# Aceinna/gnss-ins-sim

Measured on NVIDIA H100. Metric: MC-runs x timesteps/sec free_integration @100Hz, higher is better.
Workload: dtype f64

## Files before the change

### gnss_ins_sim_b200/csrc/b2ins_api.cu

```cuda
#include <cmath>
#include <cstdarg>
#include <cstdio>
#include <cstdlib>
#include <cstring>
#include <limits>
#include <vector>

#include "../../include/b2ins.h"
#include "allan_kernel.cuh"
#include "internal.h"
#include "noise_kernel.cuh"
#include "pathgen_host.h"
#include "psd_kernel.cuh"
#include "gps_kernel.cuh"
#include "ekf_kernel.cuh"
#include "stats_kernel.cuh"

#ifdef B2INS_SINGLE_TU
#define B2_RF 0
#define B2_PLAIN_NAME launch_mc_plain_rf0
#define B2_SPEC_NAME launch_mc_spec_rf0
#include "mc_plain_launch.cuh"
#include "mc_spec_launch.cuh"
#undef B2_RF
// ... 933 lines not shown
  if (rc != B2INS_OK) return rc;
  CU_CHECK(cudaMemcpyAsync(avar, dav.p, static_cast<size_t>(nseries) * ntau * sizeof(double),
                           cudaMemcpyDeviceToHost, st.s));
  CU_CHECK(cudaMemcpyAsync(tau, dtau.p, static_cast<size_t>(ntau) * sizeof(double),
                           cudaMemcpyDeviceToHost, st.s));
  CU_CHECK(cudaStreamSynchronize(st.s));
  return B2INS_OK;
}

int b2ins_psd_series_len(int64_t n) { return n > 0 ? psd_series_len(n) : 0; }

int64_t b2ins_psd_workspace_bytes(int64_t n, int64_t runs) {
  if (n <= 0 || runs <= 0) return 16;
  const int64_t L = psd_series_len(n) / 2 + 1;
  return runs * 3 * L * 2 * static_cast<int64_t>(sizeof(double)) + 8192 * 16 + 64;
}

int b2ins_psd_series_f64(double fs, int64_t n, int64_t runs, int sensor, int table_len,
                         const double* freq, const double* sxx3, uint64_t seed,
                         int64_t run_offset, double* series, void* workspace, void* stream) {
  ARG_CHECK(fs > 0.0 && n > 0 && runs >= 0, "bad fs/n/runs");
  ARG_CHECK(sensor == 0 || sensor == 1, "sensor must be 0 (accel) or 1 (gyro)");
  ARG_CHECK(table_len >= 2, "the PSD table needs at least two rows");
  if (runs == 0) return B2INS_OK;
  ARG_CHECK(freq && sxx3 && series && workspace, "null buffer");
  ARG_CHECK(runs * 3 <= 65535, "at most 21845 runs per call (grid.y)");
  PsdParams p;
  p.fs = fs;
  p.runs = runs;
  p.run_offset = run_offset;
  p.N = psd_series_len(n);
  p.L = p.N / 2 + 1;
  p.L0 = table_len;
  p.sensor = sensor;
  p.interp = (table_len != p.L) ? 1 : 0;
  p.k0 = static_cast<uint32_t>(seed);
  p.k1 = static_cast<uint32_t>(seed >> 32);
  p.freq = freq;
  p.sxx = sxx3;
  p.ab = static_cast<double*>(workspace);
  p.series = series;
  cudaStream_t s = static_cast<cudaStream_t>(stream);
  dim3 g1((p.L + kPsdThreads - 1) / kPsdThreads, static_cast<unsigned>(runs * 3));
  psd_phase_kernel<<<g1, kPsdThreads, 0, s>>>(p);
  int bluestein = 0;
  static const bool no_fft = std::getenv("B2INS_PSD_DIRECT") != nullptr;
  const int P = no_fft ? 0 : psd_fft_plan(p.N, &bluestein);
  if (P == 0) {
    dim3 g2((p.N + kPsdThreads - 1) / kPsdThreads, static_cast<unsigned>(runs * 3));
    psd_synth_kernel<<<g2, kPsdThreads, 0, s>>>(p);
    CU_CHECK(cudaGetLastError());
    return B2INS_OK;
  }
  PsdFftParams f;
  f.nseries = runs * 3;
  f.N = p.N;
  f.L = p.L;
  f.M = p.N / 2;
  f.P = P;
  f.logP = 0;
  while ((1 << f.logP) < P) ++f.logP;
  f.bluestein = bluestein;
  f.ab = p.ab;
  uintptr_t tail = reinterpret_cast<uintptr_t>(p.ab + runs * 3 * static_cast<int64_t>(p.L) * 2);
  tail = (tail + 15) & ~static_cast<uintptr_t>(15);
  f.bhat = reinterpret_cast<double2*>(tail);
  f.series = series;
  const size_t smem = static_cast<size_t>(P) * 16 + static_cast<size_t>(P / 2) * 16;
  static int attr_dev = -1;
  int dev = 0;
  CU_CHECK(cudaGetDevice(&dev));
  if (attr_dev != dev) {
    CU_CHECK(cudaFuncSetAttribute(psd_fft_kernel, cudaFuncAttributeMaxDynamicSharedMemorySize, 8192 * 24));
    CU_CHECK(cudaFuncSetAttribute(psd_chirp_kernel, cudaFuncAttributeMaxDynamicSharedMemorySize, 8192 * 24));
    attr_dev = dev;
  }
  if (bluestein) psd_chirp_kernel<<<1, kFftThreads, smem, s>>>(f);
  const int64_t grid = f.nseries < 2 * sm_count() ? f.nseries : 2 * sm_count();
  psd_fft_kernel<<<static_cast<unsigned>(grid), kFftThreads, smem, s>>>(f);
  CU_CHECK(cudaGetLastError());
  return B2INS_OK;
}

int64_t b2ins_path_rows(const double* motion_def, int64_t segs, double fs) {
  if (!motion_def || segs <= 0 || !(fs > 0.0)) return -1;
  return b2ins_host::path_rows(motion_def, segs, fs);
}

int64_t b2ins_path_gen_host(const double* ini, const double* motion_def, int64_t segs, double fs,
                            double osr, double fs_gps, double fs_odo, const double* mobility,
                            int ref_frame, int64_t cap, double* imu, double* nav, double* gps,
                            int64_t* gps_rows, double* odo) {
  if (!ini || !motion_def || !mobility || !imu || !nav || segs <= 0 || !(fs > 0.0) || !(osr >= 1.0) ||
      (ref_frame != 0 && ref_frame != 1) || (gps && !(fs_gps > 0.0))) {
    fail(B2INS_ERR_ARG, "bad argument to b2ins_path_gen_host");
    return -1;
  }
  return b2ins_host::path_gen(ini, motion_def, segs, fs, osr, fs_gps, fs_odo, mobility, ref_frame,
                              cap, imu, nav, gps, gps_rows, odo);
}

__global__ void dfma_rate_kernel(double* out, int iters) {
  double a0 = threadIdx.x * 1e-9, a1 = a0 + 1, a2 = a0 + 2, a3 = a0 + 3, a4 = a0 + 4,
         a5 = a0 + 5, a6 = a0 + 6, a7 = a0 + 7;
  const double m = 1.0000001, c = 1e-9;
  for (int i = 0; i < iters; ++i) {
    a0 = fma(a0, m, c); a1 = fma(a1, m, c); a2 = fma(a2, m, c); a3 = fma(a3, m, c);
    a4 = fma(a4, m, c); a5 = fma(a5, m, c); a6 = fma(a6, m, c); a7 = fma(a7, m, c);
  }
  out[static_cast<size_t>(blockIdx.x) * blockDim.x + threadIdx.x] = a0 + a1 + a2 + a3 + a4 + a5 + a6 + a7;
}

int b2ins_diag_auto_lanes(int64_t runs, int fused, int sm_count_arg) {
  return auto_lanes(runs < 1 ? 1 : runs, fused != 0, sm_count_arg);
}

int b2ins_diag_mc_shape(int lanes_per_run, int ref_frame, int* shape3) {
  ARG_CHECK(shape3, "null output");
  ARG_CHECK(lanes_per_run == 1 || lanes_per_run == 2 || lanes_per_run == 4 || lanes_per_run == 8 ||
                lanes_per_run == 16 || lanes_per_run == 32, "lanes_per_run must be 1,2,4,8,16 or 32");
  McShape sh = default_shape(lanes_per_run, ref_frame);
  shape_override(&sh);
  shape3[0] = sh.spec ? sh.P : 0;
  shape3[1] = sh.spec ? sh.WI : 0;
  shape3[2] = (sh.spec && sh.split) ? 1 : 0;
  return B2INS_OK;
}

int b2ins_diag_dfma_rate(double* dfma_per_s) {
  ARG_CHECK(dfma_per_s, "null output");
  const int blocks = sm_count() * 8, threads = 256, iters = 8000;
  DevBuf out;
  CU_CHECK(out.alloc(sizeof(double) * blocks * threads));
  cudaEvent_t e0, e1;
  CU_CHECK(cudaEventCreate(&e0));
  CU_CHECK(cudaEventCreate(&e1));
  float best = 1e30f;
  for (int rep = 0; rep < 4; ++rep) {
    CU_CHECK(cudaEventRecord(e0, nullptr));
    dfma_rate_kernel<<<blocks, threads>>>(out.d(), iters);
    CU_CHECK(cudaEventRecord(e1, nullptr));
    CU_CHECK(cudaEventSynchronize(e1));
    float ms = 0.f;
    CU_CHECK(cudaEventElapsedTime(&ms, e0, e1));
    if (rep > 0 && ms < best) best = ms;
  }
  cudaEventDestroy(e0);
  cudaEventDestroy(e1);
  *dfma_per_s = static_cast<double>(blocks) * threads * iters * 8.0 / (best * 1e-3);
  return B2INS_OK;
}

#ifdef B2INS_PHASE_CLOCKS
int b2ins_diag_phase_clocks(unsigned long long* out8, int reset) {
  if (out8) cudaMemcpyFromSymbol(out8, g_phase_clocks, sizeof(unsigned long long) * 8);
  if (reset) {
    unsigned long long z[8] = {0, 0, 0, 0, 0, 0, 0, 0};
    cudaMemcpyToSymbol(g_phase_clocks, z, sizeof(z));
  }
  return B2INS_OK;
}
#endif

}
```

### gnss_ins_sim_b200/csrc/mc_av_kernel.cuh

```cuda
#pragma once
#include "mc_spec_kernel.cuh"

namespace b2ins {

constexpr int kAvRound = 8;
template <int G>
struct AvShape {
  static constexpr int kHalves = (32 / G) / 4;
  static constexpr int kProd = 6 * kHalves;
  static constexpr int kWarps = (G == 4) ? 16 : 12;
  static constexpr int kSync = 32 * (2 + kProd);
};
__device__ constexpr int kAvRole8[12] = {-1, -2, 0, 1, -3, 2, 3, 4, -3, 5, -3, -3};
__device__ constexpr int kAvRole4[16] = {-1, -2, 0, 1, 2, 3, 4, 5, -3, 6, 7, 8, -3, 9, 10, 11};

template <int G>
struct AvSmem {
  alignas(128) double gyro[kStagesFast][kTile * 3];
  alignas(128) double accel[kStagesFast][kTile * 3];
  alignas(16) SampleSlot slot[3][kAvRound / G][32];
  alignas(16) double ring[2][kAvRound][32 / G][6];
  alignas(8) uint64_t full[kStagesFast];
  alignas(8) uint64_t empty[kStagesFast];
};

template <int G>
__global__ void __launch_bounds__(AvShape<G>::kWarps * 32, 1) mc_av_kernel(const __grid_constant__ McParams p) {
  static_assert(G == 4 || G == 8, "groups of 4 or 8 lanes");
  constexpr int kRunsPerCta = 32 / G;
  constexpr int kProd = AvShape<G>::kProd;
  constexpr int kAvSync = AvShape<G>::kSync;
  __shared__ AvSmem<G> sm;
  const int lane = threadIdx.x & 31;
  const int pwarp = threadIdx.x >> 5;
  const int role_w = (G == 4) ? kAvRole4[pwarp] : kAvRole8[pwarp];
  const bool is_a = role_w == -1, is_v = role_w == -2, is_p = role_w >= 0;
  const int pp = is_p ? role_w : 0;
  const int j = is_p ? (lane & 7) : lane % G;
  const int grp = is_p ? (pp / 6) * 4 + (lane >> 3) : lane / G;
  const int64_t run_raw = static_cast<int64_t>(blockIdx.x) * kRunsPerCta + grp;
  const bool active = run_raw < p.runs;
  const int64_t run = active ? run_raw : p.runs - 1;
  const int64_t grun = p.run_offset + run;
  const uint32_t run_lo = static_cast<uint32_t>(grun), run_hi = static_cast<uint32_t>(grun >> 32);
  const bool dump = active && run < p.dump_runs;
  const bool warp_dumps = __any_sync(0xffffffffu, dump);
  const int64_t num_tiles = (p.n + kTile - 1) / kTile;
  const int issuer = 2 * 32;
  auto stage_sync = [&]() { asm volatile("bar.sync 1, %0;" ::"n"(kAvSync) : "memory"); };

  if (threadIdx.x == 0) {
    for (int s = 0; s < kStagesFast; ++s) {
      mbar_init(&sm.full[s], 1);
      mbar_init(&sm.empty[s], kProd);
    }
    mbar_fence_init();
  }
  __syncthreads();
  if (!is_a && !is_v && !is_p) return;
  const int64_t rounds = (p.n + kAvRound - 1) / kAvRound;

  if (is_p) {
    if (threadIdx.x == issuer)
      for (int s = 0; s < kStagesFast && s < num_tiles; ++s) spec_issue_tile(sm, p, s, s);
    const int c = pp % 6, ax = c % 3;
    const bool is_acc = c < 3;
    const TriadNoise& e = is_acc ? p.accel : p.gyro;
    double carry = 0.0;
    const double apj = ipow(e.gm_a[ax], j), aG = ipow(e.gm_a[ax], kAvRound);
    double phase[3] = {0.0, 0.0, 0.0};
    if (p.gyro.vib_type == 2) {
#pragma unroll
      for (int k = 0; k < 3; ++k)
        phase[k] = (uniform01(0xFFFFFFFFu, kDrawPhase + k, run_lo, run_hi, p.k0, p.k1) * 2.0) * kPi;
    }
    const bool any_vib = (p.accel.vib_type | p.gyro.vib_type) != 0;
    for (int64_t i = 0; i < rounds + 2; ++i) {
      if (i < rounds) {
        const int64_t r0 = i * kAvRound;
        const int64_t tile = r0 / kTile;
        const int s = static_cast<int>(tile % kStagesFast);
        const int base = static_cast<int>(r0 - tile * kTile);
        const int cnt = static_cast<int>(min64(kTile, p.n - tile * kTile));
        if (base == 0) {
          if (threadIdx.x == issuer && tile >= 1 && tile - 1 + kStagesFast < num_tiles) {
            const int sp = static_cast<int>((tile - 1) % kStagesFast);
            mbar_wait(&sm.empty[sp], static_cast<uint32_t>(((tile - 1) / kStagesFast) & 1));
            spec_issue_tile(sm, p, tile - 1 + kStagesFast, sp);
          }
          mbar_wait(&sm.full[s], static_cast<uint32_t>((tile / kStagesFast) & 1));
        }
        const int buf = static_cast<int>(i % 3);
        {
          const int tj = base + j;
          const int64_t t = tile * kTile + tj;
          const bool live = tj < cnt;
          Normal2 z{0.0, 0.0};
          double m = 0.0;
          if (live) {
            z = normal_pair(static_cast<uint32_t>(t), c, run_lo, run_hi, p.k0, p.k1);
            const double ref = is_acc ? sm.accel[s][tj * 3 + ax] : sm.gyro[s][tj * 3 + ax];
            m = (ref + e.b[ax]) + e.w[ax] * z.z1;
            if (any_vib)
              m += vib_term(e, ax, is_acc ? 0 : 1, static_cast<uint32_t>(t), run_lo, run_hi, p.k0, p.k1, run, phase);
          }
          const double d = gm_block<kAvRound>(e.gm_b[ax] * z.z0, e.gm_a[ax], apj, aG, j, carry);
          m += d + e.wd[ax] * z.z0;
          int64_t row;
          if (warp_dumps && dump && live && p.out_gyro && dump_row(p, t, &row))
            (is_acc ? p.out_accel : p.out_gyro)[run * p.osr + row * p.ost + ax * p.osc] = m;
          SampleSlot& mine = sm.slot[buf][j / G][grp * G + (j % G)];
          if (is_acc) mine.a[ax] = m; else mine.g[ax] = m;
        }
        if (base + kAvRound >= cnt) {
          __syncwarp();
          if (lane == 0) mbar_arrive(&sm.empty[s]);
        }
      }
      if (i <= rounds) stage_sync();
    }
    return;
  }

  NavState st0;
  {
    const int64_t irun = p.ini_offset + run;
    const int64_t set = (irun < p.ini_sets) ? irun : 0;
    nav_init<1>(st0, p.ini + set * p.ini_rows, p.ini_rows, p.dt);
  }

  if (is_a) {
    AttState a;
    a.yaw = st0.yaw; a.pitch = st0.pitch; a.roll = st0.roll;
    a.sc = st0.sc;
    a.icp = st0.icp;
    if (dump && j == 0 && p.out_att) {
      const int64_t o = run * p.osr;
      p.out_att[o] = a.yaw;
      p.out_att[o + p.osc] = a.pitch;
      p.out_att[o + 2 * p.osc] = a.roll;
      if (p.out_quat) write_quat(p.out_quat + run * p.dump_rows * 4, a.yaw, a.pitch, a.roll);
    }
    for (int64_t i = 0; i < rounds + 2; ++i) {
      if (i >= 1 && i <= rounds) {
        const int64_t r0 = (i - 1) * kAvRound;
        const int sbuf = static_cast<int>((i - 1) % 3), rbuf = static_cast<int>((i - 1) & 1);
        const int kmax = static_cast<int>(min64(kAvRound, p.n - 1 - r0));
        auto a_step = [&](int k) {
          const SampleSlot& sl = sm.slot[sbuf][k / G][lane - j + (k % G)];
          const Vec3 w{sl.g[0], sl.g[1], sl.g[2]};
          att_step(a, w, p.dt, ((r0 + k + 1) & (kResync - 1)) == 0);
          if (j == 0) {
            double* o = sm.ring[rbuf][k][grp];
            reinterpret_cast<double2*>(o)[0] = make_double2(a.sc.sy, a.sc.cy);
            reinterpret_cast<double2*>(o)[1] = make_double2(a.sc.sp, a.sc.cp);
            reinterpret_cast<double2*>(o)[2] = make_double2(a.sc.sr, a.sc.cr);
          }
          int64_t row;
          if (warp_dumps && dump && j == 0 && p.out_att && dump_row(p, r0 + k + 1, &row)) {
            const int64_t o = run * p.osr + row * p.ost;
            const double y = wrap_once(a.yaw), r = wrap_once(a.roll);
            p.out_att[o] = y;
            p.out_att[o + p.osc] = a.pitch;
            p.out_att[o + 2 * p.osc] = r;
            if (p.out_quat) write_quat(p.out_quat + (run * p.dump_rows + row) * 4, y, a.pitch, r);
          }
        };
        if (warp_dumps || kmax < kAvRound) {
#pragma unroll 1
          for (int k = 0; k < kmax; ++k) a_step(k);
        } else {
#pragma unroll 1
          for (int kb = 0; kb < kAvRound; kb += 4) {
            bool redo = ((r0 + kb) & (kResync - 1)) + 4 >= kResync;
            if (!redo) {
              const AttState saved = a;
              bool cold = false;
#pragma unroll
              for (int k = 0; k < 4; ++k) {
                const SampleSlot& sl = sm.slot[sbuf][(kb + k) / G][lane - j + ((kb + k) % G)];
                const Vec3 w{sl.g[0], sl.g[1], sl.g[2]};
                cold |= att_step<true>(a, w, p.dt, false);
                if (j == 0) {
                  double* o = sm.ring[rbuf][kb + k][grp];
                  reinterpret_cast<double2*>(o)[0] = make_double2(a.sc.sy, a.sc.cy);
                  reinterpret_cast<double2*>(o)[1] = make_double2(a.sc.sp, a.sc.cp);
                  reinterpret_cast<double2*>(o)[2] = make_double2(a.sc.sr, a.sc.cr);
                }
              }
              redo = __any_sync(0xffffffffu, cold);
              if (__builtin_expect(redo, 0)) a = saved;
            }
            if (redo) {
#pragma unroll 1
              for (int k = 0; k < 4; ++k) a_step(kb + k);
            }
          }
        }
      }
      if (i <= rounds) stage_sync();
    }
    if (active && j == 0) {
      const double* r = p.ref_nav + (p.n - 1) * 9;
      if (p.end_err) {
        double* e = p.end_err + run * 9;
        e[0] = angle_range_pi(a.yaw - r[0]);
        e[1] = angle_range_pi(a.pitch - r[1]);
        e[2] = angle_range_pi(a.roll - r[2]);
      }
      if (p.end_state) {
        double* e = p.end_state + run * 9;
        e[0] = wrap_once(a.yaw); e[1] = a.pitch; e[2] = wrap_once(a.roll);
      }
    }
    return;
  }

  VelState v;
  v.vel_b = st0.vel_b;
  v.vel = st0.vel;
  v.pos = st0.pos;
  v.gdt = st0.g * p.dt;
  SinCos3 old = st0.sc;
  if (dump && j == 0 && p.out_att) {
    const int64_t o = run * p.osr;
    p.out_pos[o] = v.pos.x;
    p.out_pos[o + p.osc] = v.pos.y;
    p.out_pos[o + 2 * p.osc] = v.pos.z;
    p.out_vel[o] = v.vel.x;
    p.out_vel[o + p.osc] = v.vel.y;
    p.out_vel[o + 2 * p.osc] = v.vel.z;
  }
  for (int64_t i = 0; i < rounds + 2; ++i) {
    if (i >= 2) {
      const int64_t r0 = (i - 2) * kAvRound;
      const int sbuf = static_cast<int>((i - 2) % 3), rbuf = static_cast<int>((i - 2) & 1);
      const int kmax = static_cast<int>(min64(kAvRound, p.n - 1 - r0));
      auto v_step = [&](int k, bool hist) {
        const SampleSlot& sl = sm.slot[sbuf][k / G][lane - j + (k % G)];
        const Vec3 w{sl.g[0], sl.g[1], sl.g[2]};
        const Vec3 f{sl.a[0], sl.a[1], sl.a[2]};
        const double2* o = reinterpret_cast<const double2*>(sm.ring[rbuf][k][grp]);
        const double2 q0 = o[0], q1 = o[1], q2 = o[2];
        SinCos3 now;
        now.sy = q0.x; now.cy = q0.y; now.sp = q1.x; now.cp = q1.y; now.sr = q2.x; now.cr = q2.y;
        vel_step(v, w, f, old, now, p.dt);
        old = now;
        int64_t row;
        if (hist && dump && j == 0 && p.out_att && dump_row(p, r0 + k + 1, &row)) {
          const int64_t oo = run * p.osr + row * p.ost;
          p.out_pos[oo] = v.pos.x;
          p.out_pos[oo + p.osc] = v.pos.y;
          p.out_pos[oo + 2 * p.osc] = v.pos.z;
          p.out_vel[oo] = v.vel.x;
          p.out_vel[oo + p.osc] = v.vel.y;
          p.out_vel[oo + 2 * p.osc] = v.vel.z;
        }
      };
      if (warp_dumps || kmax < kAvRound) {
#pragma unroll 1
        for (int k = 0; k < kmax; ++k) v_step(k, true);
      } else {
#pragma unroll 1
        for (int kb = 0; kb < kAvRound; kb += 4) {
#pragma unroll
          for (int k = 0; k < 4; ++k) v_step(kb + k, false);
        }
      }
    }
    if (i <= rounds) stage_sync();
  }
  if (active && j == 0) {
    const double* r = p.ref_nav + (p.n - 1) * 9;
    if (p.end_err) {
      double* e = p.end_err + run * 9;
      e[3] = v.pos.x - r[3];
      e[4] = v.pos.y - r[4];
      e[5] = v.pos.z - r[5];
      e[6] = v.vel.x - r[6];
      e[7] = v.vel.y - r[7];
      e[8] = v.vel.z - r[8];
    }
    if (p.end_state) {
      double* e = p.end_state + run * 9;
      e[3] = v.pos.x; e[4] = v.pos.y; e[5] = v.pos.z;
      e[6] = v.vel.x; e[7] = v.vel.y; e[8] = v.vel.z;
    }
  }
}

}
```

### gnss_ins_sim_b200/csrc/mc_kernel.cuh

```cuda
#pragma once
#include "mech.cuh"

namespace b2ins {

#ifdef B2INS_PHASE_CLOCKS
__device__ unsigned long long g_phase_clocks[8];
#define B2_CLK(var) const long long var = clock64()
#define B2_ACC(i, t0, t1) \
  if ((threadIdx.x & 31) == 0) atomicAdd(&g_phase_clocks[i], static_cast<unsigned long long>((t1) - (t0)))
#else
#define B2_CLK(var)
#define B2_ACC(i, t0, t1)
#endif

constexpr int kWarps = 4;
constexpr int kThreads = kWarps * 32;
constexpr int kTile = 128;
constexpr int kStagesFast = 3;
template <bool PROC>
struct Stages {
  static constexpr int value = PROC ? 2 : kStagesFast;
};

struct TriadNoise {
  double b[3];
  double gm_a[3];
  double gm_b[3];
  double wd[3];
  double w[3];
  int vib_type;
  int series_len;
  double vib_amp[3];
  double vib_w;
  const double* series;
};

struct McParams {
  int64_t n, runs, run_offset, ini_offset;
  double dt;
  int earth_rot;
  uint32_t k0, k1;
  TriadNoise gyro, accel;
  const double* ref_gyro;
  const double* ref_accel;
  const double* ref_nav;
  const double* ini;
  int ini_sets, ini_rows;
  const double* fed_gyro;
  const double* fed_accel;
  int64_t sr, st, sc;
  int algo;
  const double* ref_odo;
  double odo_scale, odo_stdv;
  const double* fed_odo;
  int64_t so_r, so_t;
  double* out_att;
  double* out_pos;
  double* out_vel;
  double* out_gyro;
  double* out_accel;
  double* out_odo;
  double* out_quat;
  int64_t osr, ost, osc;
  int64_t dump_runs;
  int64_t dump_stride;
  int64_t dump_rows;
  double* end_err;
  double* end_state;
  double* proc_stats;
  int64_t stats_start;
  int debug;
};

struct alignas(16) SampleSlot {
  double g[3], a[3];
};

template <bool PROC>
struct TileSmem {
  static constexpr int kStages = Stages<PROC>::value;
  alignas(128) double gyro[kStages][kTile * 3];
  alignas(128) double accel[kStages][kTile * 3];
  alignas(128) double nav[kStages][PROC ? kTile * 9 : 2];
  alignas(16) SampleSlot slot[kWarps][32];
  alignas(8) uint64_t full[kStages];
  alignas(8) uint64_t empty[kStages];
};

template <bool FED, bool PROC>
__device__ __forceinline__ void issue_tile(TileSmem<PROC>& sm, const McParams& p, int64_t tile, int s) {
  const int64_t t0 = tile * kTile;
  const uint32_t cnt = static_cast<uint32_t>(min64(kTile, p.n - t0));
  uint32_t tx = 0;
  if (!FED) tx += 2u * ((cnt * 24u) & ~15u);
  if (PROC) tx += (cnt * 72u) & ~15u;
  if (!FED) {
    if ((cnt * 24u) & 8u) {
      const uint32_t o = ((cnt * 24u) & ~15u) / 8;
      sm.gyro[s][o] = p.ref_gyro[t0 * 3 + o];
      sm.accel[s][o] = p.ref_accel[t0 * 3 + o];
    }
  }
  if (PROC) {
    if ((cnt * 72u) & 8u) {
      const uint32_t o = ((cnt * 72u) & ~15u) / 8;
      sm.nav[s][o] = p.ref_nav[t0 * 9 + o];
    }
  }
  mbar_arrive_expect_tx(&sm.full[s], tx);
  if (!FED) {
    const uint32_t b = (cnt * 24u) & ~15u;
    if (b) {
      bulk_g2s(sm.gyro[s], p.ref_gyro + t0 * 3, b, &sm.full[s]);
      bulk_g2s(sm.accel[s], p.ref_accel + t0 * 3, b, &sm.full[s]);
    }
  }
  if (PROC) {
    const uint32_t b = (cnt * 72u) & ~15u;
    if (b) bulk_g2s(sm.nav[s], p.ref_nav + t0 * 9, b, &sm.full[s]);
  }
}

__device__ __forceinline__ double vib_term(const TriadNoise& e, int c, int sensor, uint32_t t,
                                           uint32_t run_lo, uint32_t run_hi, uint32_t k0,
                                           uint32_t k1, int64_t run_local, const double* phase) {
  if (e.vib_type == 1) {
    const Normal2 zv = normal_pair(t, kDrawVib + c, run_lo, run_hi, k0, k1);
    return e.vib_amp[c] * (sensor == 0 ? zv.z0 : zv.z1);
  }
  if (e.vib_type == 2) {
    const double arg = e.vib_w * static_cast<double>(t) + (sensor == 0 ? 0.0 : phase[c]);
    return e.vib_amp[c] * sin(arg);
  }
  if (e.vib_type == 3)
    return e.series[(run_local * 3 + c) * e.series_len + (t % static_cast<uint32_t>(e.series_len))];
  return 0.0;
}

template <class P>
__device__ __forceinline__ void noisy_sample(const P& p, const double* ref_a3,
                                             const double* ref_g3, uint32_t t, uint32_t run_lo,
                                             uint32_t run_hi, int64_t run_local,
                                             const double* phase, double* ma, double* mg,
                                             double* za, double* zg) {
  Normal2 z[6];
#pragma unroll
  for (int c = 0; c < 6; ++c) z[c] = normal_pair(t, c, run_lo, run_hi, p.k0, p.k1);
#pragma unroll
  for (int c = 0; c < 3; ++c) {
    za[c] = z[c].z0;
    zg[c] = z[3 + c].z0;
    ma[c] = (ref_a3[c] + p.accel.b[c]) + p.accel.w[c] * z[c].z1;
    mg[c] = (ref_g3[c] + p.gyro.b[c]) + p.gyro.w[c] * z[3 + c].z1;
  }
  if (p.accel.vib_type | p.gyro.vib_type) {
#pragma unroll
    for (int c = 0; c < 3; ++c) {
      ma[c] += vib_term(p.accel, c, 0, t, run_lo, run_hi, p.k0, p.k1, run_local, phase);
      mg[c] += vib_term(p.gyro, c, 1, t, run_lo, run_hi, p.k0, p.k1, run_local, phase);
// ... 365 lines not shown
```

### gnss_ins_sim_b200/csrc/mc_plain_launch.cuh

```cuda
#include "internal.h"

namespace b2ins {
namespace {

template <int G>
void launch_g(const McParams& p, bool fed, bool proc, cudaStream_t s) {
  const int64_t runs_per_cta = static_cast<int64_t>(kWarps) * (32 / G);
  const unsigned grid = static_cast<unsigned>((p.runs + runs_per_cta - 1) / runs_per_cta);
  if (fed) {
    if (proc)
      mc_kernel<G, B2_RF, true, true><<<grid, kThreads, 0, s>>>(p);
    else
      mc_kernel<G, B2_RF, true, false><<<grid, kThreads, 0, s>>>(p);
  } else {
    if (proc)
      mc_kernel<G, B2_RF, false, true><<<grid, kThreads, 0, s>>>(p);
    else
      mc_kernel<G, B2_RF, false, false><<<grid, kThreads, 0, s>>>(p);
  }
}

}

void B2_PLAIN_NAME(const McParams& p, int lanes, bool fed, bool proc, cudaStream_t s) {
  switch (lanes) {
    case 1: launch_g<1>(p, fed, proc, s); break;
    case 2: launch_g<2>(p, fed, proc, s); break;
    case 4: launch_g<4>(p, fed, proc, s); break;
    case 8: launch_g<8>(p, fed, proc, s); break;
    case 16: launch_g<16>(p, fed, proc, s); break;
    default: launch_g<32>(p, fed, proc, s); break;
  }
}

}
```

### gnss_ins_sim_b200/csrc/mc_spec_launch.cuh

```cuda
#include "internal.h"
#include "mc_spec_kernel.cuh"
#if B2_RF == 1
#include "mc_av_kernel.cuh"
#endif

namespace b2ins {
namespace {

template <int G, int P, int WI, bool SPLIT, int MINB>
void launch_one(const McParams& p, cudaStream_t s) {
  const int64_t runs_per_cta = static_cast<int64_t>(WI) * (32 / G);
  const unsigned grid = static_cast<unsigned>((p.runs + runs_per_cta - 1) / runs_per_cta);
  mc_spec_kernel<G, B2_RF, P, WI, SPLIT, MINB><<<grid, SpecShape<G, P, WI>::kThreads, 0, s>>>(p);
}

#if B2_RF == 1
template <int G>
void launch_av(const McParams& p, cudaStream_t s) {
  const int64_t runs_per_cta = 32 / G;
  const unsigned grid = static_cast<unsigned>((p.runs + runs_per_cta - 1) / runs_per_cta);
  mc_av_kernel<G><<<grid, AvShape<G>::kWarps * 32, 0, s>>>(p);
}
#endif

}

bool B2_SPEC_NAME(const McParams& p, const McShape& sh, cudaStream_t s) {
  const int key = sh.G * 1000 + sh.P * 100 + sh.WI * 10 + (sh.split ? 1 : 0);
  switch (key) {
    case 1310: launch_one<1, 3, 1, false, 3>(p, s); return true;
    case 1610: launch_one<1, 6, 1, false, 2>(p, s); return true;
    case 2310: launch_one<2, 3, 1, false, 3>(p, s); return true;
    case 2610: launch_one<2, 6, 1, false, 2>(p, s); return true;
    case 4310: launch_one<4, 3, 1, false, 2>(p, s); return true;
    case 4311: launch_one<4, 3, 1, true, 2>(p, s); return true;
    case 4610: launch_one<4, 6, 1, false, 1>(p, s); return true;
    case 4611: launch_one<4, 6, 1, true, 1>(p, s); return true;
#if B2_RF == 1
    case 4620: launch_av<4>(p, s); return true;
    case 8620: launch_av<8>(p, s); return true;
#endif
    case 8120: launch_one<8, 1, 2, false, 2>(p, s); return true;
    case 8610: launch_one<8, 6, 1, false, 1>(p, s); return true;
    case 16140: launch_one<16, 1, 4, false, 1>(p, s); return true;
    case 16141: launch_one<16, 1, 4, true, 1>(p, s); return true;
    case 32141: launch_one<32, 1, 4, true, 1>(p, s); return true;
    default: return false;
  }
}

}
```

### gnss_ins_sim_b200/csrc/mech.cuh

```cuda
#pragma once
#include "common.cuh"

#ifdef B2INS_HOST_TEST
#define B2_DEV __host__ __device__ __forceinline__
#else
#define B2_DEV __device__ __forceinline__
#endif

namespace b2ins {

struct Vec3 {
  double x, y, z;
};

struct Dcm {
  double c00, c01, c02, c10, c11, c12, c20, c21, c22;
};

struct SinCos3 {
  double sy, cy, sp, cp, sr, cr;
};

B2_DEV void sincos_angle(double x, double* s, double* c) {
  sincos_bounded(fabs(x) <= 1.0e6 ? x : 0.0, s, c);
// ... 145 lines not shown
    s.sc.sr = __shfl_sync(0xffffffffu, sv, 2, 4);
    s.sc.cr = __shfl_sync(0xffffffffu, cv, 2, 4);
    if (RF == 0) {
      s.sl = __shfl_sync(0xffffffffu, sv, 3, 4);
      s.cl = __shfl_sync(0xffffffffu, cv, 3, 4);
    }
#endif
  }
}

template <int RF>
B2_DEV void nav_init(NavState& s, const double* __restrict__ ini,
                                         int ini_rows, double dt) {
  const double lat = ini[0], lon = ini[1], alt = ini[2];
  s.vel_b = Vec3{ini[3], ini[4], ini[5]};
  s.yaw = ini[6];
  s.pitch = ini[7];
  s.roll = ini[8];
  s.sl = s.cl = 0.0;
  if (RF == 1) {
    s.pos = lla2ecef(lat, lon, alt);
    s.g = (ini_rows > 9) ? ini[9] : geo_param(lat, alt).g;
    s.fixed_g = true;
  } else {
    s.pos = Vec3{lat, lon, alt};
    s.fixed_g = ini_rows > 9;
    s.g = s.fixed_g ? ini[9] : 0.0;
  }
  refresh_trig<RF, false>(s, 0);
  s.icp = rcp_nr(s.sc.cp) * dt;
  const Dcm c = dcm_from_sincos(s.sc);
  s.vel = mul_t(c, s.vel_b);
}

template <int RF>
B2_DEV void resync_exact(NavState& s) {
  double y0 = s.yaw, y1 = s.pitch, y2 = s.roll;
  const bool hi = y1 > kHalfPi, lo = y1 < -kHalfPi;
  y1 = hi ? (kPi - y1) : (lo ? (-kPi - y1) : y1);
  const bool flip = hi || lo;
  y0 = flip ? y0 + kPi : y0;
  y2 = flip ? y2 + kPi : y2;
  s.yaw = wrap_once(y0);
  s.pitch = y1;
  s.roll = wrap_once(y2);
  refresh_trig<RF, false>(s, 0);
}

template <int RF, bool SPLIT, int ODO = 0, bool SPEC = false>
B2_DEV bool nav_step(NavState& s, const Vec3& gyro, const Vec3& accel, double dt, bool earth_rot, int role,
                     bool resync, bool odo_rt = false) {
  const bool odo = (ODO == 2) ? odo_rt : (ODO == 1);
  const Vec3 vel_old = s.vel;
  Vec3 w = gyro;
  Vec3 cgdt, wxv;
  Vec3 fa, cor;
  double g = s.g, dlat = 0.0;
  if (RF == 1) {
    const double gdt = s.g * dt;
    const double cpg = s.sc.cp * gdt;
    cgdt = Vec3{-s.sc.sp * gdt, cpg * s.sc.sr, cpg * s.sc.cr};
    wxv = cross3(gyro, s.vel_b);
  } else {
    const GeoParam p = geo_param_sc(s.sl, s.cl, s.pos.z);
    const double rm_e = p.rm + s.pos.z;
    const double rn_e = p.rn + s.pos.z;
    g = s.fixed_g ? s.g : p.g;
    const double inv_rn = rcp_nr(rn_e), inv_rm = rcp_nr(rm_e), inv_cl = rcp_nr(p.cl);
    const Vec3 w_en{s.vel.y * inv_rn, -s.vel.x * inv_rm, -s.vel.y * p.sl * inv_cl * inv_rn};
    Vec3 w_ie{0.0, 0.0, 0.0};
    if (earth_rot) {
      w_ie.x = kWie * p.cl;
      w_ie.z = -kWie * p.sl;
    }
    const Vec3 w_sum{w_en.x + w_ie.x, w_en.y + w_ie.y, w_en.z + w_ie.z};
    const Vec3 cw = rot_n2b(s.sc, w_sum);
    w = Vec3{gyro.x - cw.x, gyro.y - cw.y, gyro.z - cw.z};
    fa = rot_b2n(s.sc, accel);
    const Vec3 w2{2 * w_ie.x + w_en.x, 2 * w_ie.y + w_en.y, 2 * w_ie.z + w_en.z};
    cor = cross3(w2, s.vel);
    dlat = vel_old.x * inv_rm * dt;
    s.pos.x += dlat;
    s.pos.y += vel_old.y * inv_rn * inv_cl * dt;
    s.pos.z += (-vel_old.z) * dt;
  }
  const double t = b2_fma(w.z, s.sc.cr, w.y * s.sc.sr);
  const double dy = t * s.icp;
  const double dp = b2_fma(w.y, s.sc.cr, -(w.z * s.sc.sr)) * dt;
  const double dr = b2_fma(dy, s.sc.sp, w.x * dt);
  s.yaw += dy;
  s.pitch += dp;
  s.roll += dr;
  const bool cold = resync | !(fabs(s.pitch) <= kHalfPi) | !(fabs(dy) <= kRotMax) |
                    !(fabs(dp) <= kRotMax) | !(fabs(dr) <= kRotMax) |
                    (RF == 0 && !(fabs(dlat) <= kLatRotMax));
  if (!SPLIT) {
    rot_small(s.sc.sy, s.sc.cy, dy);
    rot_small(s.sc.sp, s.sc.cp, dp);
    rot_small(s.sc.sr, s.sc.cr, dr);
    if (RF == 0) rot_tiny(s.sl, s.cl, dlat);
  } else {
    double sv = s.sc.sr, cv = s.sc.cr, d = dr;
    if (role == 0) { sv = s.sc.sy; cv = s.sc.cy; d = dy; }
    if (role == 1) { sv = s.sc.sp; cv = s.sc.cp; d = dp; }
    if (RF == 0 && role == 3) { sv = s.sl; cv = s.cl; d = dlat; }
    rot_small(sv, cv, d);
#ifdef __CUDA_ARCH__
    s.sc.sy = __shfl_sync(0xffffffffu, sv, 0, 4);
    s.sc.cy = __shfl_sync(0xffffffffu, cv, 0, 4);
    s.sc.sp = __shfl_sync(0xffffffffu, sv, 1, 4);
    s.sc.cp = __shfl_sync(0xffffffffu, cv, 1, 4);
    s.sc.sr = __shfl_sync(0xffffffffu, sv, 2, 4);
    s.sc.cr = __shfl_sync(0xffffffffu, cv, 2, 4);
    if (RF == 0) {
      s.sl = __shfl_sync(0xffffffffu, sv, 3, 4);
      s.cl = __shfl_sync(0xffffffffu, cv, 3, 4);
    }
#endif
  }
  if (!SPEC) {
    if (__builtin_expect(cold, 0)) resync_exact<RF>(s);
  }
  s.icp = rcp_nr(s.sc.cp) * dt;
  if (RF == 1) {
    if (odo) {
      s.vel_b = Vec3{accel.x, 0.0, 0.0};
    } else {
      s.vel_b.x = b2_fma(-wxv.x, dt, b2_fma(accel.x, dt, s.vel_b.x) + cgdt.x);
      s.vel_b.y = b2_fma(-wxv.y, dt, b2_fma(accel.y, dt, s.vel_b.y) + cgdt.y);
      s.vel_b.z = b2_fma(-wxv.z, dt, b2_fma(accel.z, dt, s.vel_b.z) + cgdt.z);
    }
    s.vel = rot_b2n(s.sc, s.vel_b);
    s.pos.x = b2_fma(vel_old.x, dt, s.pos.x);
    s.pos.y = b2_fma(vel_old.y, dt, s.pos.y);
    s.pos.z = b2_fma(vel_old.z, dt, s.pos.z);
  } else {
    if (odo) {
      s.vel = rot_b2n(s.sc, Vec3{accel.x, 0.0, 0.0});
    } else {
      s.vel.x = b2_fma(fa.x - cor.x, dt, vel_old.x);
      s.vel.y = b2_fma(fa.y - cor.y, dt, vel_old.y);
      s.vel.z = b2_fma(fa.z + g - cor.z, dt, vel_old.z);
    }
  }
  return cold;
}

struct AttState {
  double yaw, pitch, roll;
  SinCos3 sc;
  double icp;
};

template <bool SPEC = false>
B2_DEV bool att_step(AttState& s, const Vec3& w, double dt, bool resync) {
  const double t = b2_fma(w.z, s.sc.cr, w.y * s.sc.sr);
  const double dy = t * s.icp;
  const double dp = b2_fma(w.y, s.sc.cr, -(w.z * s.sc.sr)) * dt;
  const double dr = b2_fma(dy, s.sc.sp, w.x * dt);
  s.yaw += dy;
  s.pitch += dp;
  s.roll += dr;
  const bool cold = resync | !(fabs(s.pitch) <= kHalfPi) | !(fabs(dy) <= kRotMax) |
                    !(fabs(dp) <= kRotMax) | !(fabs(dr) <= kRotMax);
  rot_small(s.sc.sy, s.sc.cy, dy);
  rot_small(s.sc.sp, s.sc.cp, dp);
  rot_small(s.sc.sr, s.sc.cr, dr);
  if (!SPEC && __builtin_expect(cold, 0)) {
    NavState n;
    n.yaw = s.yaw; n.pitch = s.pitch; n.roll = s.roll;
    n.pos = Vec3{0.0, 0.0, 0.0};
    resync_exact<1>(n);
    s.yaw = n.yaw; s.pitch = n.pitch; s.roll = n.roll;
    s.sc = n.sc;
  }
  s.icp = rcp_nr(s.sc.cp) * dt;
  return cold;
}

struct VelState {
  Vec3 vel_b, vel, pos;
  double gdt;
};

B2_DEV void vel_step(VelState& s, const Vec3& gyro, const Vec3& accel, const SinCos3& old, const SinCos3& now,
                     double dt) {
  const double cpg = old.cp * s.gdt;
  const Vec3 cgdt{-old.sp * s.gdt, cpg * old.sr, cpg * old.cr};
  const Vec3 wxv = cross3(gyro, s.vel_b);
  const Vec3 vel_old = s.vel;
  s.vel_b.x = b2_fma(-wxv.x, dt, b2_fma(accel.x, dt, s.vel_b.x) + cgdt.x);
  s.vel_b.y = b2_fma(-wxv.y, dt, b2_fma(accel.y, dt, s.vel_b.y) + cgdt.y);
  s.vel_b.z = b2_fma(-wxv.z, dt, b2_fma(accel.z, dt, s.vel_b.z) + cgdt.z);
  s.vel = rot_b2n(now, s.vel_b);
  s.pos.x = b2_fma(vel_old.x, dt, s.pos.x);
  s.pos.y = b2_fma(vel_old.y, dt, s.pos.y);
  s.pos.z = b2_fma(vel_old.z, dt, s.pos.z);
}

}
```

Before: 5.627 billion.

## Streamline AV producer loop and speculate attitude through resync blocks

```diff
diff --git a/gnss_ins_sim_b200/csrc/b2ins_api.cu b/gnss_ins_sim_b200/csrc/b2ins_api.cu
--- a/gnss_ins_sim_b200/csrc/b2ins_api.cu
+++ b/gnss_ins_sim_b200/csrc/b2ins_api.cu
@@ -1109,10 +1109,10 @@
 }
 
 #ifdef B2INS_PHASE_CLOCKS
-int b2ins_diag_phase_clocks(unsigned long long* out8, int reset) {
-  if (out8) cudaMemcpyFromSymbol(out8, g_phase_clocks, sizeof(unsigned long long) * 8);
+int b2ins_diag_phase_clocks(unsigned long long* out16, int reset) {
+  if (out16) cudaMemcpyFromSymbol(out16, g_phase_clocks, sizeof(unsigned long long) * kPhaseClocks);
   if (reset) {
-    unsigned long long z[8] = {0, 0, 0, 0, 0, 0, 0, 0};
+    unsigned long long z[kPhaseClocks] = {};
     cudaMemcpyToSymbol(g_phase_clocks, z, sizeof(z));
   }
   return B2INS_OK;
diff --git a/gnss_ins_sim_b200/csrc/mc_av_kernel.cuh b/gnss_ins_sim_b200/csrc/mc_av_kernel.cuh
--- a/gnss_ins_sim_b200/csrc/mc_av_kernel.cuh
+++ b/gnss_ins_sim_b200/csrc/mc_av_kernel.cuh
@@ -1,4 +1,6 @@
 #pragma once
+#include <type_traits>
+
 #include "mc_spec_kernel.cuh"
 
 namespace b2ins {
@@ -13,6 +15,7 @@
 };
 __device__ constexpr int kAvRole8[12] = {-1, -2, 0, 1, -3, 2, 3, 4, -3, 5, -3, -3};
 __device__ constexpr int kAvRole4[16] = {-1, -2, 0, 1, 2, 3, 4, 5, -3, 6, 7, 8, -3, 9, 10, 11};
+
 
 template <int G>
 struct AvSmem {
@@ -56,6 +59,14 @@
     }
     mbar_fence_init();
   }
+#ifdef B2INS_PHASE_CLOCKS
+  if (p.debug) {
+    for (int q = threadIdx.x; q < static_cast<int>(sizeof(sm.slot) / 8); q += blockDim.x)
+      reinterpret_cast<double*>(sm.slot)[q] = 0.0;
+    for (int q = threadIdx.x; q < static_cast<int>(sizeof(sm.ring) / 8); q += blockDim.x)
+      reinterpret_cast<double*>(sm.ring)[q] = 0.0;
+  }
+#endif
   __syncthreads();
   if (!is_a && !is_v && !is_p) return;
   const int64_t rounds = (p.n + kAvRound - 1) / kAvRound;
@@ -66,8 +77,9 @@
     const int c = pp % 6, ax = c % 3;
     const bool is_acc = c < 3;
     const TriadNoise& e = is_acc ? p.accel : p.gyro;
+    const double eb = e.b[ax], ew = e.w[ax], ewd = e.wd[ax], ga = e.gm_a[ax], gb = e.gm_b[ax];
     double carry = 0.0;
-    const double apj = ipow(e.gm_a[ax], j), aG = ipow(e.gm_a[ax], kAvRound);
+    const double apj = ipow(ga, j), aG = ipow(ga, kAvRound);
     double phase[3] = {0.0, 0.0, 0.0};
     if (p.gyro.vib_type == 2) {
 #pragma unroll
@@ -75,50 +87,82 @@
         phase[k] = (uniform01(0xFFFFFFFFu, kDrawPhase + k, run_lo, run_hi, p.k0, p.k1) * 2.0) * kPi;
     }
     const bool any_vib = (p.accel.vib_type | p.gyro.vib_type) != 0;
-    for (int64_t i = 0; i < rounds + 2; ++i) {
-      if (i < rounds) {
-        const int64_t r0 = i * kAvRound;
-        const int64_t tile = r0 / kTile;
-        const int s = static_cast<int>(tile % kStagesFast);
-        const int base = static_cast<int>(r0 - tile * kTile);
-        const int cnt = static_cast<int>(min64(kTile, p.n - tile * kTile));
+    const double* ref0 = (is_acc ? sm.accel[0] : sm.gyro[0]) + j * 3 + ax;
+    SampleSlot& slot0 = sm.slot[0][j / G][grp * G + (j % G)];
+    double* out0 = (is_acc ? slot0.a : slot0.g) + ax;
+    constexpr int kSlotSet = static_cast<int>(sizeof(sm.slot[0]) / sizeof(double));
+    const int nrounds = static_cast<int>(rounds);
+    const int ntiles = static_cast<int>(num_tiles);
+    auto produce = [&](auto slow) {
+      constexpr bool kSlow = decltype(slow)::value;
+      int tile = 0, s = 0, base = 0, ref_off = 0, out_off = 0;
+      uint32_t parity = 0, t0 = 0;
+      int cnt = static_cast<int>(min64(kTile, p.n));
+      for (int i = 0; i < nrounds; ++i) {
         if (base == 0) {
-          if (threadIdx.x == issuer && tile >= 1 && tile - 1 + kStagesFast < num_tiles) {
-            const int sp = static_cast<int>((tile - 1) % kStagesFast);
-            mbar_wait(&sm.empty[sp], static_cast<uint32_t>(((tile - 1) / kStagesFast) & 1));
+          if (threadIdx.x == issuer && tile >= 1 && tile - 1 + kStagesFast < ntiles) {
+            const int sp = (s == 0) ? kStagesFast - 1 : s - 1;
+            mbar_wait(&sm.empty[sp], (s == 0) ? parity ^ 1u : parity);
             spec_issue_tile(sm, p, tile - 1 + kStagesFast, sp);
           }
-          mbar_wait(&sm.full[s], static_cast<uint32_t>((tile / kStagesFast) & 1));
-        }
-        const int buf = static_cast<int>(i % 3);
+          B2_CLK(cw0);
+          mbar_wait(&sm.full[s], parity);
+          B2_CLK(cw1);
+          B2_ACC(13, cw0, cw1);
+        }
+        B2_CLK(cp0);
+#ifdef B2INS_PHASE_CLOCKS
+        if (!(p.debug & 1))
+#endif
         {
           const int tj = base + j;
-          const int64_t t = tile * kTile + tj;
+          const uint32_t t = t0 + static_cast<uint32_t>(tj);
           const bool live = tj < cnt;
           Normal2 z{0.0, 0.0};
           double m = 0.0;
           if (live) {
-            z = normal_pair(static_cast<uint32_t>(t), c, run_lo, run_hi, p.k0, p.k1);
-            const double ref = is_acc ? sm.accel[s][tj * 3 + ax] : sm.gyro[s][tj * 3 + ax];
-            m = (ref + e.b[ax]) + e.w[ax] * z.z1;
-            if (any_vib)
-              m += vib_term(e, ax, is_acc ? 0 : 1, static_cast<uint32_t>(t), run_lo, run_hi, p.k0, p.k1, run, phase);
-          }
-          const double d = gm_block<kAvRound>(e.gm_b[ax] * z.z0, e.gm_a[ax], apj, aG, j, carry);
-          m += d + e.wd[ax] * z.z0;
+            z = normal_pair(t, c, run_lo, run_hi, p.k0, p.k1);
+            m = (ref0[ref_off] + eb) + ew * z.z1;
+            if (kSlow && any_vib)
+              m += vib_term(e, ax, is_acc ? 0 : 1, t, run_lo, run_hi, p.k0, p.k1, run, phase);
+          }
+          const double d = gm_block<kAvRound>(gb * z.z0, ga, apj, aG, j, carry);
+          m += d + ewd * z.z0;
           int64_t row;
-          if (warp_dumps && dump && live && p.out_gyro && dump_row(p, t, &row))
+          if (kSlow && warp_dumps && dump && live && p.out_gyro && dump_row(p, t, &row))
             (is_acc ? p.out_accel : p.out_gyro)[run * p.osr + row * p.ost + ax * p.osc] = m;
-          SampleSlot& mine = sm.slot[buf][j / G][grp * G + (j % G)];
-          if (is_acc) mine.a[ax] = m; else mine.g[ax] = m;
-        }
+          out0[out_off] = m;
+        }
+        B2_CLK(cp1);
+        B2_ACC(14, cp0, cp1);
         if (base + kAvRound >= cnt) {
           __syncwarp();
           if (lane == 0) mbar_arrive(&sm.empty[s]);
-        }
-      }
-      if (i <= rounds) stage_sync();
-    }
+          ++tile;
+          if (++s == kStagesFast) {
+            s = 0;
+            parity ^= 1u;
+          }
+          base = 0;
+          t0 += kTile;
+          ref_off = s * kTile * 3;
+          cnt = static_cast<int>(min64(kTile, p.n - static_cast<int64_t>(t0)));
+        } else {
+          base += kAvRound;
+          ref_off += kAvRound * 3;
+        }
+        out_off = (out_off == 2 * kSlotSet) ? 0 : out_off + kSlotSet;
+        B2_CLK(cb0);
+        stage_sync();
+        B2_CLK(cb1);
+        B2_ACC(15, cb0, cb1);
+      }
+      stage_sync();
+    };
+    if (warp_dumps || any_vib)
+      produce(std::true_type{});
+    else
+      produce(std::false_type{});
     return;
   }
 
@@ -142,20 +186,27 @@
       if (p.out_quat) write_quat(p.out_quat + run * p.dump_rows * 4, a.yaw, a.pitch, a.roll);
     }
     for (int64_t i = 0; i < rounds + 2; ++i) {
+      B2_CLK(ca0);
+#ifdef B2INS_PHASE_CLOCKS
+      if (!(p.debug & 2))
+#endif
       if (i >= 1 && i <= rounds) {
         const int64_t r0 = (i - 1) * kAvRound;
         const int sbuf = static_cast<int>((i - 1) % 3), rbuf = static_cast<int>((i - 1) & 1);
         const int kmax = static_cast<int>(min64(kAvRound, p.n - 1 - r0));
-        auto a_step = [&](int k) {
-          const SampleSlot& sl = sm.slot[sbuf][k / G][lane - j + (k % G)];
-          const Vec3 w{sl.g[0], sl.g[1], sl.g[2]};
-          att_step(a, w, p.dt, ((r0 + k + 1) & (kResync - 1)) == 0);
+        auto ring_store = [&](int k) {
           if (j == 0) {
             double* o = sm.ring[rbuf][k][grp];
             reinterpret_cast<double2*>(o)[0] = make_double2(a.sc.sy, a.sc.cy);
             reinterpret_cast<double2*>(o)[1] = make_double2(a.sc.sp, a.sc.cp);
             reinterpret_cast<double2*>(o)[2] = make_double2(a.sc.sr, a.sc.cr);
           }
+        };
+        auto a_step = [&](int k) {
+          const SampleSlot& sl = sm.slot[sbuf][k / G][lane - j + (k % G)];
+          const Vec3 w{sl.g[0], sl.g[1], sl.g[2]};
+          att_step(a, w, p.dt, ((r0 + k + 1) & (kResync - 1)) == 0);
+          ring_store(k);
           int64_t row;
           if (warp_dumps && dump && j == 0 && p.out_att && dump_row(p, r0 + k + 1, &row)) {
             const int64_t o = run * p.osr + row * p.ost;
@@ -170,35 +221,42 @@
 #pragma unroll 1
           for (int k = 0; k < kmax; ++k) a_step(k);
         } else {
+          static_assert(kAvRound % 4 == 0 && kResync % 4 == 0, "blocks of four steps");
 #pragma unroll 1
           for (int kb = 0; kb < kAvRound; kb += 4) {
-            bool redo = ((r0 + kb) & (kResync - 1)) + 4 >= kResync;
-            if (!redo) {
-              const AttState saved = a;
-              bool cold = false;
+            const AttState saved = a;
+            Vec3 w[4];
 #pragma unroll
-              for (int k = 0; k < 4; ++k) {
-                const SampleSlot& sl = sm.slot[sbuf][(kb + k) / G][lane - j + ((kb + k) % G)];
-                const Vec3 w{sl.g[0], sl.g[1], sl.g[2]};
-                cold |= att_step<true>(a, w, p.dt, false);
-                if (j == 0) {
-                  double* o = sm.ring[rbuf][kb + k][grp];
-                  reinterpret_cast<double2*>(o)[0] = make_double2(a.sc.sy, a.sc.cy);
-                  reinterpret_cast<double2*>(o)[1] = make_double2(a.sc.sp, a.sc.cp);
-                  reinterpret_cast<double2*>(o)[2] = make_double2(a.sc.sr, a.sc.cr);
-                }
-              }
-              redo = __any_sync(0xffffffffu, cold);
-              if (__builtin_expect(redo, 0)) a = saved;
+            for (int k = 0; k < 4; ++k) {
+              const SampleSlot& sl = sm.slot[sbuf][(kb + k) / G][lane - j + ((kb + k) % G)];
+              w[k] = Vec3{sl.g[0], sl.g[1], sl.g[2]};
             }
-            if (redo) {
+            bool cold = false;
+#pragma unroll
+            for (int k = 0; k < 4; ++k) {
+              cold |= att_step<true>(a, w[k], p.dt, false);
+              ring_store(kb + k);
+            }
+            B2_CLK(cr0);
+            if (__builtin_expect(__any_sync(0xffffffffu, cold), 0)) {
+              a = saved;
 #pragma unroll 1
               for (int k = 0; k < 4; ++k) a_step(kb + k);
+            } else if (((r0 + kb + 4) & (kResync - 1)) == 0) {
+              att_exact(a);
+              a.icp = rcp_nr(a.sc.cp) * p.dt;
+              ring_store(kb + 3);
             }
-          }
-        }
-      }
+            B2_CLK(cr1);
+            B2_ACC(10, cr0, cr1);
+          }
+        }
+      }
+      B2_CLK(ca1);
+      B2_ACC(8, ca0, ca1);
       if (i <= rounds) stage_sync();
+      B2_CLK(ca2);
+      B2_ACC(9, ca1, ca2);
     }
     if (active && j == 0) {
       const double* r = p.ref_nav + (p.n - 1) * 9;
@@ -232,6 +290,10 @@
     p.out_vel[o + 2 * p.osc] = v.vel.z;
   }
   for (int64_t i = 0; i < rounds + 2; ++i) {
+    B2_CLK(cv0);
+#ifdef B2INS_PHASE_CLOCKS
+    if (!(p.debug & 4))
+#endif
     if (i >= 2) {
       const int64_t r0 = (i - 2) * kAvRound;
       const int sbuf = static_cast<int>((i - 2) % 3), rbuf = static_cast<int>((i - 2) & 1);
@@ -268,7 +330,11 @@
         }
       }
     }
+    B2_CLK(cv1);
+    B2_ACC(11, cv0, cv1);
     if (i <= rounds) stage_sync();
+    B2_CLK(cv2);
+    B2_ACC(12, cv1, cv2);
   }
   if (active && j == 0) {
     const double* r = p.ref_nav + (p.n - 1) * 9;
diff --git a/gnss_ins_sim_b200/csrc/mc_kernel.cuh b/gnss_ins_sim_b200/csrc/mc_kernel.cuh
--- a/gnss_ins_sim_b200/csrc/mc_kernel.cuh
+++ b/gnss_ins_sim_b200/csrc/mc_kernel.cuh
@@ -3,8 +3,9 @@
 
 namespace b2ins {
 
+constexpr int kPhaseClocks = 16;
 #ifdef B2INS_PHASE_CLOCKS
-__device__ unsigned long long g_phase_clocks[8];
+__device__ unsigned long long g_phase_clocks[kPhaseClocks];
 #define B2_CLK(var) const long long var = clock64()
 #define B2_ACC(i, t0, t1) \
   if ((threadIdx.x & 31) == 0) atomicAdd(&g_phase_clocks[i], static_cast<unsigned long long>((t1) - (t0)))
diff --git a/gnss_ins_sim_b200/csrc/mc_plain_launch.cuh b/gnss_ins_sim_b200/csrc/mc_plain_launch.cuh
--- a/gnss_ins_sim_b200/csrc/mc_plain_launch.cuh
+++ b/gnss_ins_sim_b200/csrc/mc_plain_launch.cuh
@@ -1,35 +1,38 @@
 #include "internal.h"
 
 namespace b2ins {
+#ifndef B2INS_MC_PLAIN_HELPERS
+#define B2INS_MC_PLAIN_HELPERS
 namespace {
 
-template <int G>
+template <int G, int RF>
 void launch_g(const McParams& p, bool fed, bool proc, cudaStream_t s) {
   const int64_t runs_per_cta = static_cast<int64_t>(kWarps) * (32 / G);
   const unsigned grid = static_cast<unsigned>((p.runs + runs_per_cta - 1) / runs_per_cta);
   if (fed) {
     if (proc)
-      mc_kernel<G, B2_RF, true, true><<<grid, kThreads, 0, s>>>(p);
+      mc_kernel<G, RF, true, true><<<grid, kThreads, 0, s>>>(p);
     else
-      mc_kernel<G, B2_RF, true, false><<<grid, kThreads, 0, s>>>(p);
+      mc_kernel<G, RF, true, false><<<grid, kThreads, 0, s>>>(p);
   } else {
     if (proc)
-      mc_kernel<G, B2_RF, false, true><<<grid, kThreads, 0, s>>>(p);
+      mc_kernel<G, RF, false, true><<<grid, kThreads, 0, s>>>(p);
     else
-      mc_kernel<G, B2_RF, false, false><<<grid, kThreads, 0, s>>>(p);
+      mc_kernel<G, RF, false, false><<<grid, kThreads, 0, s>>>(p);
   }
 }
 
 }
+#endif
 
 void B2_PLAIN_NAME(const McParams& p, int lanes, bool fed, bool proc, cudaStream_t s) {
   switch (lanes) {
-    case 1: launch_g<1>(p, fed, proc, s); break;
-    case 2: launch_g<2>(p, fed, proc, s); break;
-    case 4: launch_g<4>(p, fed, proc, s); break;
-    case 8: launch_g<8>(p, fed, proc, s); break;
-    case 16: launch_g<16>(p, fed, proc, s); break;
-    default: launch_g<32>(p, fed, proc, s); break;
+    case 1: launch_g<1, B2_RF>(p, fed, proc, s); break;
+    case 2: launch_g<2, B2_RF>(p, fed, proc, s); break;
+    case 4: launch_g<4, B2_RF>(p, fed, proc, s); break;
+    case 8: launch_g<8, B2_RF>(p, fed, proc, s); break;
+    case 16: launch_g<16, B2_RF>(p, fed, proc, s); break;
+    default: launch_g<32, B2_RF>(p, fed, proc, s); break;
   }
 }
 
diff --git a/gnss_ins_sim_b200/csrc/mc_spec_launch.cuh b/gnss_ins_sim_b200/csrc/mc_spec_launch.cuh
--- a/gnss_ins_sim_b200/csrc/mc_spec_launch.cuh
+++ b/gnss_ins_sim_b200/csrc/mc_spec_launch.cuh
@@ -1,50 +1,49 @@
 #include "internal.h"
 #include "mc_spec_kernel.cuh"
-#if B2_RF == 1
 #include "mc_av_kernel.cuh"
-#endif
 
 namespace b2ins {
+#ifndef B2INS_MC_SPEC_HELPERS
+#define B2INS_MC_SPEC_HELPERS
 namespace {
 
-template <int G, int P, int WI, bool SPLIT, int MINB>
+template <int G, int RF, int P, int WI, bool SPLIT, int MINB>
 void launch_one(const McParams& p, cudaStream_t s) {
   const int64_t runs_per_cta = static_cast<int64_t>(WI) * (32 / G);
   const unsigned grid = static_cast<unsigned>((p.runs + runs_per_cta - 1) / runs_per_cta);
-  mc_spec_kernel<G, B2_RF, P, WI, SPLIT, MINB><<<grid, SpecShape<G, P, WI>::kThreads, 0, s>>>(p);
+  mc_spec_kernel<G, RF, P, WI, SPLIT, MINB><<<grid, SpecShape<G, P, WI>::kThreads, 0, s>>>(p);
 }
 
-#if B2_RF == 1
 template <int G>
 void launch_av(const McParams& p, cudaStream_t s) {
   const int64_t runs_per_cta = 32 / G;
   const unsigned grid = static_cast<unsigned>((p.runs + runs_per_cta - 1) / runs_per_cta);
   mc_av_kernel<G><<<grid, AvShape<G>::kWarps * 32, 0, s>>>(p);
 }
-#endif
 
 }
+#endif
 
 bool B2_SPEC_NAME(const McParams& p, const McShape& sh, cudaStream_t s) {
   const int key = sh.G * 1000 + sh.P * 100 + sh.WI * 10 + (sh.split ? 1 : 0);
   switch (key) {
-    case 1310: launch_one<1, 3, 1, false, 3>(p, s); return true;
-    case 1610: launch_one<1, 6, 1, false, 2>(p, s); return true;
-    case 2310: launch_one<2, 3, 1, false, 3>(p, s); return true;
-    case 2610: launch_one<2, 6, 1, false, 2>(p, s); return true;
-    case 4310: launch_one<4, 3, 1, false, 2>(p, s); return true;
-    case 4311: launch_one<4, 3, 1, true, 2>(p, s); return true;
-    case 4610: launch_one<4, 6, 1, false, 1>(p, s); return true;
-    case 4611: launch_one<4, 6, 1, true, 1>(p, s); return true;
+    case 1310: launch_one<1, B2_RF, 3, 1, false, 3>(p, s); return true;
+    case 1610: launch_one<1, B2_RF, 6, 1, false, 2>(p, s); return true;
+    case 2310: launch_one<2, B2_RF, 3, 1, false, 3>(p, s); return true;
+    case 2610: launch_one<2, B2_RF, 6, 1, false, 2>(p, s); return true;
+    case 4310: launch_one<4, B2_RF, 3, 1, false, 2>(p, s); return true;
+    case 4311: launch_one<4, B2_RF, 3, 1, true, 2>(p, s); return true;
+    case 4610: launch_one<4, B2_RF, 6, 1, false, 1>(p, s); return true;
+    case 4611: launch_one<4, B2_RF, 6, 1, true, 1>(p, s); return true;
 #if B2_RF == 1
     case 4620: launch_av<4>(p, s); return true;
     case 8620: launch_av<8>(p, s); return true;
 #endif
-    case 8120: launch_one<8, 1, 2, false, 2>(p, s); return true;
-    case 8610: launch_one<8, 6, 1, false, 1>(p, s); return true;
-    case 16140: launch_one<16, 1, 4, false, 1>(p, s); return true;
-    case 16141: launch_one<16, 1, 4, true, 1>(p, s); return true;
-    case 32141: launch_one<32, 1, 4, true, 1>(p, s); return true;
+    case 8120: launch_one<8, B2_RF, 1, 2, false, 2>(p, s); return true;
+    case 8610: launch_one<8, B2_RF, 6, 1, false, 1>(p, s); return true;
+    case 16140: launch_one<16, B2_RF, 1, 4, false, 1>(p, s); return true;
+    case 16141: launch_one<16, B2_RF, 1, 4, true, 1>(p, s); return true;
+    case 32141: launch_one<32, B2_RF, 1, 4, true, 1>(p, s); return true;
     default: return false;
   }
 }
diff --git a/gnss_ins_sim_b200/csrc/mech.cuh b/gnss_ins_sim_b200/csrc/mech.cuh
--- a/gnss_ins_sim_b200/csrc/mech.cuh
+++ b/gnss_ins_sim_b200/csrc/mech.cuh
@@ -321,6 +321,15 @@
   double icp;
 };
 
+B2_DEV void att_exact(AttState& s) {
+  NavState n;
+  n.yaw = s.yaw; n.pitch = s.pitch; n.roll = s.roll;
+  n.pos = Vec3{0.0, 0.0, 0.0};
+  resync_exact<1>(n);
+  s.yaw = n.yaw; s.pitch = n.pitch; s.roll = n.roll;
+  s.sc = n.sc;
+}
+
 template <bool SPEC = false>
 B2_DEV bool att_step(AttState& s, const Vec3& w, double dt, bool resync) {
   const double t = b2_fma(w.z, s.sc.cr, w.y * s.sc.sr);
@@ -335,14 +344,7 @@
   rot_small(s.sc.sy, s.sc.cy, dy);
   rot_small(s.sc.sp, s.sc.cp, dp);
   rot_small(s.sc.sr, s.sc.cr, dr);
-  if (!SPEC && __builtin_expect(cold, 0)) {
-    NavState n;
-    n.yaw = s.yaw; n.pitch = s.pitch; n.roll = s.roll;
-    n.pos = Vec3{0.0, 0.0, 0.0};
-    resync_exact<1>(n);
-    s.yaw = n.yaw; s.pitch = n.pitch; s.roll = n.roll;
-    s.sc = n.sc;
-  }
+  if (!SPEC && __builtin_expect(cold, 0)) att_exact(s);
   s.icp = rcp_nr(s.sc.cp) * dt;
   return cold;
 }
```

Result: faster. 6.825 billion, median of 6 (+21.3%).
